# adahbingee/pais-mvs

Hardware: AMD Instinct MI355X
Metric: refined+expanded patches/sec (higher is better)
Workload: dtype f64

## Files before the change

include/pais_hip.h:

```cpp
#ifndef PAIS_HIP_H
#define PAIS_HIP_H

#include <stdint.h>
#include <stddef.h>

#ifdef __cplusplus
extern "C" {
#endif

#define PAIS_MAX_LEVELS 16
#define PAIS_MAX_VIS    64
#define PAIS_MAX_PARTICLES 128

#define PAIS_TYPE_SEED   0
#define PAIS_TYPE_EXPAND 1

typedef struct pais_config {
    int32_t cellSize;
    int32_t patchRadius;
    int32_t patchSize;
    int32_t minCamNum;
    double  textureVariation;
    double  visibleCorrelation;
    double  minCorrelation;
// ... 104 lines not shown
#define PAIS_COST_BACKFACING  1
#define PAIS_COST_OFF_IMAGE   2
#define PAIS_COST_WINDOW      3
#define PAIS_COST_OVERFLOW    4
#define PAIS_COST_ALL_MASKED  5
#define PAIS_PIX_COUNTED      0
#define PAIS_PIX_MASKED       1
#define PAIS_PIX_OVERFLOW     2
#define PAIS_PIX_NONE         3

typedef struct pais_cost_detail {
    double  fitness;
    double  sum_weight;
    double  sum_weighted_sad;
    double  pt[2];
    int32_t outcome, nx, ny;
    int32_t live_pixels;
    int32_t overflow_pixel;
    int32_t overflow_cam;
    int32_t ref_pos, _pad;
} pais_cost_detail;

int  pais_fitness_detail(pais_ctx *ctx, int n_states, const pais_patch_state *states,
                         int n_evals, const int32_t *state_index, const double *particles,
                         pais_cost_detail *out, double *weight, double *avg_sad, int8_t *pixel_code,
                         double *colour, double *homographies, int cam_stride);
int  pais_get_detail_stats(pais_ctx *ctx, double *kernel_ms, int64_t *launches, int64_t *evals, int reset);
size_t pais_sizeof_cost_detail(void);

int  pais_refine_batch(pais_ctx *ctx, int n, const pais_candidate *cands, pais_patch_result *out);
int  pais_refine_batch_view(pais_ctx *ctx, int n, const pais_candidate *cands, const pais_patch_result **view);
int  pais_refine_batch_begin(pais_ctx *ctx, int n, const pais_candidate *cands);
int  pais_refine_batch_end(pais_ctx *ctx, const pais_patch_result **view);

typedef struct pais_pso_run_info {
    double  range_l[3], range_u[3];
    double  init[3];
    double  ray[3];
    int32_t run;
    int32_t ref_cam, lod, num_cam;
    int32_t n_particles, max_iteration;
    int32_t iterations;
    int32_t _pad;
    int32_t cam_idx[PAIS_MAX_VIS];
} pais_pso_run_info;

typedef struct pais_pso_iter {
    double  gbest_fitness, gbest[3];
    double  iw;
    double  dispersion, velocity;
    int32_t g_idx, iteration, ended, _pad;
} pais_pso_iter;

int  pais_pso_trace_shape(pais_ctx *ctx, int n, const pais_candidate *cands, int *rows_per_run, int *particles_per_row);
int  pais_pso_trace(pais_ctx *ctx, int n, const pais_candidate *cands, int max_runs, pais_patch_result *out,
                    pais_pso_run_info *runs, pais_pso_iter *iters, double *particles);
int  pais_get_trace_stats(pais_ctx *ctx, double *kernel_ms, int64_t *launches, int64_t *evals, int reset);
size_t pais_sizeof_pso_run_info(void);
size_t pais_sizeof_pso_iter(void);

int  pais_refine_batch_open(pais_ctx *ctx, int n, const pais_candidate *cands, int iterations);
int  pais_refine_batch_enqueue(pais_ctx *ctx, int iterations);
int  pais_ctx_fork_lane(pais_ctx *parent, pais_ctx **lane);
int  pais_ctx_set_round_hint(pais_ctx *ctx, int n_round);

int  pais_refine_batch_device(pais_ctx *ctx, int n, const pais_candidate *d_cands,
// ... 87 lines not shown
```

pais_mvs_amd/_lib.py:

```python
from __future__ import annotations

import ctypes as C
import os

from . import build as _build

MAX_LEVELS = 16
MAX_VIS = 64


class Config(C.Structure):
    _fields_ = [
        ("cellSize", C.c_int32), ("patchRadius", C.c_int32), ("patchSize", C.c_int32), ("minCamNum", C.c_int32),
        ("textureVariation", C.c_double), ("visibleCorrelation", C.c_double), ("minCorrelation", C.c_double),
        ("maxFitness", C.c_double), ("lodRatio", C.c_double),
        ("minLOD", C.c_int32), ("maxLOD", C.c_int32), ("maxCellPatchNum", C.c_int32), ("_pad0", C.c_int32),
        ("reduceNormalRange", C.c_double),
        ("adaptiveDistanceEnable", C.c_int32), ("adaptiveDifferenceEnable", C.c_int32),
        ("adaptiveGradientEnable", C.c_int32), ("_pad1", C.c_int32),
        ("distWeighting", C.c_double), ("diffWeighting", C.c_double), ("gradientWeighting", C.c_double),
        ("neighborRadius", C.c_double), ("neighborRadiusScalar", C.c_double), ("minRegionRatio", C.c_double),
        ("depthRangeScalar", C.c_double),
        ("particleNum", C.c_int32), ("maxIteration", C.c_int32), ("expansionStrategy", C.c_int32), ("_pad2", C.c_int32),
    ]
# ... 107 lines not shown
    L.pais_last_error.restype = C.c_char_p
    for n in ("pais_sizeof_config", "pais_sizeof_camera_desc", "pais_sizeof_candidate", "pais_sizeof_patch_result",
              "pais_sizeof_view_state", "pais_sizeof_view_result", "pais_sizeof_cost_detail",
              "pais_sizeof_pso_run_info", "pais_sizeof_pso_iter"):
        getattr(L, n).restype = C.c_size_t
    assert L.pais_sizeof_config() == C.sizeof(Config), (L.pais_sizeof_config(), C.sizeof(Config))
    assert L.pais_sizeof_camera_desc() == C.sizeof(CameraDesc)
    assert L.pais_sizeof_candidate() == C.sizeof(Candidate)
    assert L.pais_sizeof_patch_result() == C.sizeof(PatchResult), (L.pais_sizeof_patch_result(), C.sizeof(PatchResult))
    assert L.pais_sizeof_view_state() == C.sizeof(ViewState), (L.pais_sizeof_view_state(), C.sizeof(ViewState))
    assert L.pais_sizeof_view_result() == C.sizeof(ViewResult), (L.pais_sizeof_view_result(), C.sizeof(ViewResult))
    assert L.pais_sizeof_cost_detail() == C.sizeof(CostDetail), (L.pais_sizeof_cost_detail(), C.sizeof(CostDetail))
    assert L.pais_sizeof_pso_run_info() == C.sizeof(PsoRunInfo), (L.pais_sizeof_pso_run_info(), C.sizeof(PsoRunInfo))
    assert L.pais_sizeof_pso_iter() == C.sizeof(PsoIter), (L.pais_sizeof_pso_iter(), C.sizeof(PsoIter))
    L.pais_ctx_create.restype = C.c_int
    L.pais_ctx_create.argtypes = [C.POINTER(Config), C.c_int, C.POINTER(CameraDesc), C.c_int, C.c_uint64,
                                  C.POINTER(C.c_void_p)]
    L.pais_ctx_set_config.argtypes = [C.c_void_p, C.POINTER(Config)]
    L.pais_ctx_set_neighbor_radius.argtypes = [C.c_void_p, C.c_double]
    L.pais_ctx_destroy.argtypes = [C.c_void_p]
    L.pais_ctx_destroy.restype = None
    L.pais_ctx_stream.restype = C.c_void_p
    L.pais_ctx_stream.argtypes = [C.c_void_p]
    L.pais_ctx_synchronize.argtypes = [C.c_void_p]
    L.pais_fitness_batch.argtypes = [C.c_void_p, C.c_int, C.POINTER(PatchState), C.c_int, C.POINTER(C.c_int32),
                                     C.POINTER(C.c_double), C.POINTER(C.c_double)]
    L.pais_refine_batch.argtypes = [C.c_void_p, C.c_int, C.POINTER(Candidate), C.POINTER(PatchResult)]
    L.pais_refine_batch_device.argtypes = [C.c_void_p, C.c_int, C.c_void_p, C.c_void_p, C.c_int, C.c_int]
    L.pais_refine_batch_begin.argtypes = [C.c_void_p, C.c_int, C.POINTER(Candidate)]
    L.pais_refine_batch_open.argtypes = [C.c_void_p, C.c_int, C.POINTER(Candidate), C.c_int]
    L.pais_refine_batch_enqueue.argtypes = [C.c_void_p, C.c_int]
    L.pais_ctx_set_round_hint.argtypes = [C.c_void_p, C.c_int]
    L.pais_refine_batch_end.argtypes = [C.c_void_p, C.POINTER(C.POINTER(PatchResult))]
    L.pais_ctx_fork_lane.argtypes = [C.c_void_p, C.POINTER(C.c_void_p)]
    L.pais_get_kernel_stats.argtypes = [C.c_void_p, C.POINTER(KernelStats), C.c_int]
    L.pais_ctx_set_fine_timing.argtypes = [C.c_void_p, C.c_int]
    L.pais_neighbor_count.argtypes = [C.c_void_p, C.c_int, C.POINTER(C.c_double), C.c_double, C.POINTER(C.c_int32), C.POINTER(C.c_double)]
    L.pais_ncc_batch.argtypes = [C.c_void_p, C.c_int, C.POINTER(ViewState), C.POINTER(ViewResult), C.POINTER(C.c_double), C.c_int]
    L.pais_fitness_detail.argtypes = [C.c_void_p, C.c_int, C.POINTER(PatchState), C.c_int, C.POINTER(C.c_int32),
                                      C.POINTER(C.c_double), C.POINTER(CostDetail), C.POINTER(C.c_double), C.POINTER(C.c_double),
                                      C.POINTER(C.c_int8), C.POINTER(C.c_double), C.POINTER(C.c_double), C.c_int]
    L.pais_pso_trace.argtypes = [C.c_void_p, C.c_int, C.POINTER(Candidate), C.c_int, C.POINTER(PatchResult), C.c_void_p, C.c_void_p,
                                 C.POINTER(C.c_double)]
    L.pais_pso_trace_shape.argtypes = [C.c_void_p, C.c_int, C.POINTER(Candidate), C.POINTER(C.c_int), C.POINTER(C.c_int)]
    L.pais_get_trace_stats.argtypes = [C.c_void_p, C.POINTER(C.c_double), C.POINTER(C.c_int64), C.POINTER(C.c_int64), C.c_int]
    L.pais_get_detail_stats.argtypes = [C.c_void_p, C.POINTER(C.c_double), C.POINTER(C.c_int64), C.POINTER(C.c_int64), C.c_int]
    L.pais_get_ncc_stats.argtypes = [C.c_void_p, C.POINTER(C.c_double), C.POINTER(C.c_int64), C.POINTER(C.c_int64), C.c_int]
    L.pais_rand31.restype = C.c_uint32
    L.pais_rand31.argtypes = [C.c_uint64, C.c_uint64, C.c_uint32, C.c_uint32]
    L.pais_child_key.restype = C.c_uint64
    L.pais_child_key.argtypes = [C.c_uint64, C.c_int, C.c_int, C.c_int]
    _lib = L
    return L


def check(rc: int, what: str = ""):
    if rc != 0:
        raise RuntimeError("%s failed (%d): %s" % (what or "pais call", rc, load().pais_last_error().decode()))
```

pais_mvs_amd/csrc/pais_capi.hip:

```cpp
#include <hip/hip_runtime.h>
#include <limits.h>
#include <math.h>
#include <stdarg.h>
#include <stddef.h>
#include <stdio.h>
#include <stdlib.h>
#include <string.h>

#include <string>
#include <utility>
#include <vector>
#include <algorithm>

#include "../../include/pais_hip.h"
#include "pais_dev.hpp"
#include "pais_host.hpp"
#include "pais_internal.h"

static thread_local std::string g_err;
static int fail(const char *what, hipError_t e)
{
    char buf[512];
    snprintf(buf, sizeof(buf), "%s: %s", what, hipGetErrorString(e));
    g_err = buf;
// ... 132 lines not shown
    DevBuf<double> d_nbC;
    DevBuf<int32_t> d_nbN;
    bool fineTiming = false;
    std::vector<EventPair> evPso, evBegin, evAfter, evEval, evEval2;
    std::vector<EventPair> evFree;
    double psoMs = 0, beginMs = 0, afterMs = 0, evalMs = 0, eval2Ms = 0;
    hipEvent_t refEv = nullptr;
    std::vector<std::pair<float, float>> eval2Intervals;
    int64_t psoLaunches = 0, evalLaunches = 0, eval2Launches = 0, tileLaunches = 0, ringLaunches = 0;
    pais_ctx *parent = nullptr;
    std::vector<pais_ctx *> lanes;
    int openBatch = -1;
    double ringPerCam = 1843.0;
    int ringMode = 1;
    int preMode = 1;
    DevBuf<double> d_pre;
    DevBuf<unsigned> d_ring;
    DevBuf<unsigned> d_ringCtl;
    PinBuf<unsigned> h_ringCtl;
    DevBuf<int> d_arrive;
    bool ringUsed = false;
    bool ringSuppressed = false;
    bool ringSuppressOnce = false;
    int ringPendingN = 0;
    double ringTimeoutMs = 10000.0;
    long ringSeedAbove = 0;
    size_t ringMaxBytes = (size_t)512 << 20;
    int64_t ringFallbacks = 0;
    std::vector<EventPair> evRing;
    double ringMs = 0;
    PassPlan plan;
    bool planDone = true;
    int roundHint = 0;
};

static void build_gauss(const pais_config &cfg, std::vector<double> &g)
{
    const int S = cfg.patchSize, r = cfg.patchRadius;
    g.assign((size_t)S * S, 0.0);
    const double sigma = cfg.distWeighting;
    const double s2 = 1.0 / (2.0 * sigma * sigma);
    const double s = 1.0 / (2.0 * M_PI * sigma * sigma);
    for (int x = 0; x < S; ++x)
        for (int y = 0; y < S; ++y) {
            double e = -(pow((double)(x - r), 2) + pow((double)(y - r), 2)) * s2;
            g[(size_t)x * S + y] = s * exp(e);
        }
    double n = 0;
    for (size_t i = 0; i < g.size(); ++i) n += g[i];
    const double inv = 1.0 / n;
    for (size_t i = 0; i < g.size(); ++i) g[i] = g[i] * inv;
}

static int apply_config(pais_ctx *ctx, const pais_config *cfg)
{
    pais_config c = *cfg;
    c.patchSize = (c.patchRadius << 1) + 1;
    if (c.patchRadius < 1 || c.patchRadius > 127) return fail_msg("patchRadius out of range");
    if (c.particleNum < 1 || c.particleNum * 2 > PAIS_MAX_PARTICLES) return fail_msg("particleNum out of range");
    if (c.maxLOD < 0 || c.maxLOD >= PAIS_MAX_LEVELS) return fail_msg("maxLOD out of range");
    std::vector<double> g;
    build_gauss(c, g);
    if (ctx->d_gauss) HIPCHK(hipStreamSynchronize(ctx->stream));
    HIPCHK(ctx->d_gauss.alloc(g.size() * sizeof(double)));
    HIPCHK(hipMemcpy(ctx->d_gauss, g.data(), g.size() * sizeof(double), hipMemcpyHostToDevice));
    ctx->sc.cfg = c;
// ... 187 lines not shown
    HIPCHK(ctx->d_stat.alloc(sizeof(unsigned long long) * 24));
    HIPCHK(hipMemset(ctx->d_stat, 0, sizeof(unsigned long long) * 24));
    ctx->stat = ctx->d_stat;
    HIPCHK(ctx->h_counters.alloc(sizeof(int) * 4));
    HIPCHK(ctx->d_ringCtl.alloc(PAIS_RING_CTL_BYTES * PAIS_RINGS));
    HIPCHK(hipMemset(ctx->d_ringCtl, 0, PAIS_RING_CTL_BYTES * PAIS_RINGS));
    HIPCHK(ctx->h_ringCtl.alloc(PAIS_RING_CTL_BYTES * PAIS_RINGS));
    memset(ctx->h_ringCtl, 0, PAIS_RING_CTL_BYTES * PAIS_RINGS);
    ctx->splitAbove = 3L * ctx->numCUs * 12;
    env_int("PAIS_EVAL_PARTS", ctx->evalParts, 1, 4);
    if (ctx->evalParts == 3) ctx->evalParts = 0;
    env_real("PAIS_PART_FILL", ctx->partFill, true);
    env_int("PAIS_SPLIT_ABOVE", ctx->splitAbove, 1);
    env_int("PAIS_PSO_MINPER", ctx->psoMinPer, 1, INT_MAX);
    env_int("PAIS_PSO_STREAMS", ctx->psoStreams, 1, 16);
    env_int("PAIS_PSO_RING", ctx->ringMode, INT_MIN, INT_MAX);
    env_int("PAIS_PRE_SETUP", ctx->preMode, INT_MIN, INT_MAX);
    env_real("PAIS_RING_PER_CAM", ctx->ringPerCam);
    env_int("PAIS_RING_SEED_ABOVE", ctx->ringSeedAbove);
    long ringMaxMB = 0;
    env_int("PAIS_RING_MAX_MB", ringMaxMB, 1);
    if (ringMaxMB) ctx->ringMaxBytes = (size_t)ringMaxMB << 20;
    env_int("PAIS_TILE", ctx->tileMode, INT_MIN, INT_MAX);
    env_flag("PAIS_TILE_DEBUG", ctx->tileDebug);
    env_flag("PAIS_TILE_VERIFY", ctx->tileVerify);
    env_int("PAIS_TILE_STRIP2", ctx->tileStrip2, 2, INT_MAX);
    env_int("PAIS_TILE_STRIP1", ctx->tileStrip1, 1, INT_MAX);
    env_flag("PAIS_TILE_FORCE_NS1", ctx->tileForceNs1);
    env_int("PAIS_TILE_SPLIT", ctx->tileSplit, INT_MIN, INT_MAX);
    if (ctx->tileSplit < 0) ctx->tileSplit = 0;
    env_int("PAIS_TILE_STRIP_SPLIT", ctx->tileStripSplit, 1, INT_MAX);
    env_int("PAIS_TILE_ABOVE", ctx->tileAbove, 1);
    env_flag("PAIS_FINE_TIMING", ctx->fineTiming);
    if (const char *e = getenv("PAIS_ARITH")) ctx->arithLiteral = (strcmp(e, "literal") == 0);
    if (const char *e = getenv("PAIS_RING_TIMEOUT_MS")) {
        const double v = atof(e);
        if (v == 0.0 && e[0] == '0') ctx->ringTimeoutMs = 0.0;
        else if (v >= 1.0 && v <= 600000.0) ctx->ringTimeoutMs = v;
        else fprintf(stderr, "pais: PAIS_RING_TIMEOUT_MS=%s ignored (0, or 1 .. 600000 ms)\n", e);
    }
    HIPCHK(hipEventCreateWithFlags(&ctx->forkEv, hipEventDisableTiming));
    for (int i = 0; i + 1 < ctx->psoStreams; ++i) {
        hipStream_t st; hipEvent_t ev;
        HIPCHK(hipStreamCreateWithFlags(&st, hipStreamNonBlocking));
        HIPCHK(hipEventCreateWithFlags(&ev, hipEventDisableTiming));
        ctx->sub.push_back(st);
        ctx->subDone.push_back(ev);
    }
    return 0;
}

extern "C" void pais_ctx_destroy(pais_ctx *ctx)
{
    if (!ctx) return;
    (void)hipSetDevice(ctx->device);
    if (ctx->parent) {
        auto &v = ctx->parent->lanes;
        for (size_t i = 0; i < v.size(); ++i)
            if (v[i] == ctx) { v.erase(v.begin() + (long)i); break; }
        ctx->parent = nullptr;
    }
    while (!ctx->lanes.empty()) {
        pais_ctx *l = ctx->lanes.back();
        ctx->lanes.pop_back();
        l->parent = nullptr;
        pais_ctx_destroy(l);
    }
    if (ctx->stream) (void)hipStreamSynchronize(ctx->stream);
    for (auto *v : {&ctx->evPso, &ctx->evBegin, &ctx->evAfter, &ctx->evEval, &ctx->evEval2, &ctx->evRing, &ctx->evFree})
        for (auto &p : *v) { (void)hipEventDestroy(p.a); (void)hipEventDestroy(p.b); }
    for (auto st : ctx->sub) (void)hipStreamDestroy(st);
    for (auto ev : ctx->subDone) (void)hipEventDestroy(ev);
    if (ctx->forkEv) (void)hipEventDestroy(ctx->forkEv);
    if (ctx->refEv) (void)hipEventDestroy(ctx->refEv);
    pais_launch::ring_profile_print();
    if (ctx->stream) (void)hipStreamDestroy(ctx->stream);
    delete ctx;
}

extern "C" int pais_ctx_set_config(pais_ctx *ctx, const pais_config *cfg)
{
    if (!ctx || !cfg) return fail_msg("pais_ctx_set_config: bad argument");
    HIPCHK(hipSetDevice(ctx->device));
    if (cfg->adaptiveGradientEnable && !ctx->d_edge && !ctx->edgesOnTheFly)
        return fail_msg("adaptiveGradientEnable needs the gradient weighting enabled at create time (edge pyramids or their on-the-fly statistics)");
    if (ctx->parent) return fail_msg("pais_ctx_set_config: a lane takes its configuration from its parent");
    for (pais_ctx *l : ctx->lanes) HIPCHK(hipStreamSynchronize(l->stream));
    int rc = apply_config(ctx, cfg);
    if (rc) return rc;
    for (pais_ctx *l : ctx->lanes) {
        l->sc.cfg = ctx->sc.cfg;
        l->sc.gauss = ctx->sc.gauss;
        for (int i = 0; i < PAIS_MAX_LEVELS; ++i) l->sc.lodScale[i] = ctx->sc.lodScale[i];
    }
    return 0;
}

extern "C" int pais_ctx_fork_lane(pais_ctx *parent, pais_ctx **out)
{
    if (!parent || !out) return fail_msg("pais_ctx_fork_lane: bad argument");
    if (parent->parent) return fail_msg("pais_ctx_fork_lane: a lane cannot be forked");
    HIPCHK(hipSetDevice(parent->device));
// ... 484 lines not shown
            if (P.useTile) ctx->tileLaunches++;
            if (P.trace) {
                const TraceOut &t = *P.trace;
                const size_t slot0 = (size_t)q.lo * t.maxRuns;
                HIPCHK(pais_launch::pso_step_trace(sc, P.d_out + q.lo, stp, q.hi - q.lo, P.Nmax, ctx->stat, t.runs + slot0, t.iters + slot0 * t.rows,
                                                   t.particles ? t.particles + slot0 * t.rows * P.Nmax * 11 : nullptr, t.maxRuns, t.rows, q.st));
                P.trace->launches++;
            } else if (!P.useIter)
                HIPCHK(pais_launch::pso_step(sc, P.d_out + q.lo, stp, q.hi - q.lo, P.Nmax, ctx->stat, q.st, ctx->d_evalBlocks + P.EB * (size_t)q.lo,
                                             P.usePre ? (double *)((unsigned char *)ctx->d_pre.p + P.PB * (size_t)q.lo) : nullptr, P.Kmax));
        }
    }
    if (tev.a) {
        if (timed_end(ctx, tev)) return -2;
        P.trace->ev->push_back(tev);
    }
    if (itEnd > P.itNext) P.itNext = itEnd;
    return 0;
}

static int pass_join(pais_ctx *ctx, PassPlan &P)
{
    for (int sI = 1; sI < P.S; ++sI) {
        bool used = false;
        for (int k = 0; k < P.nSl; ++k) used = used || (P.sl[k].st == ctx->sub[sI - 1]);
        if (!used) continue;
        HIPCHK(hipEventRecord(ctx->subDone[sI - 1], ctx->sub[sI - 1]));
        HIPCHK(hipStreamWaitEvent(ctx->stream, ctx->subDone[sI - 1], 0));
    }
    P.S = 1;
    return 0;
}

static int pass_close(pais_ctx *ctx, PassPlan &P)
{
    const DevScene &sc = ctx->sc;
    for (int k = 0; k < P.nSl; ++k) {
        const PassPlan::Slice &q = P.sl[k];
        if (P.useIter)
            HIPCHK(pais_launch::pso_iter(sc, ctx->d_psoStates, ctx->d_active, P.cnt + 2, q.lo, q.hi, P.Nmax, P.Kmax, P.d_out,
                                         ctx->stat, P.maxIt + 1, 1, q.parts, ctx->d_evalBlocks, ctx->d_win, q.st));
    }
    if (pass_join(ctx, P)) return -2;
    if (P.tp.end()) return -2;
    ctx->psoLaunches++;
    Timed ta;
    if (ta.begin(ctx, ctx->stream, &ctx->evAfter)) return -2;
    HIPCHK(pais_launch::after(sc, P.d_out, P.n, ctx->d_hp, P.afterGrid, P.cnt, ctx->stat, P.Kmax, ctx->d_ratios, P.nextCnt, ctx->stream));
    if (ta.end()) return -2;
    return 0;
}

static int batch_setup(pais_ctx *ctx, PassPlan &P, int n, const pais_candidate *d_cands, pais_patch_result *d_out, int max_num_cam, int has_seeds)
{
    HIPCHK(hipSetDevice(ctx->device));
    const DevScene &sc = ctx->sc;
    int Kmax = max_num_cam > 0 ? max_num_cam : sc.numCams;
    if (Kmax > PAIS_MAX_VIS) Kmax = PAIS_MAX_VIS;
    if (Kmax > sc.numCams) Kmax = sc.numCams;
    if (Kmax < 1) Kmax = 1;
    const int Nmax = has_seeds ? sc.cfg.particleNum * 2 : sc.cfg.particleNum;
    const int S2 = sc.cfg.patchSize * sc.cfg.patchSize;
    const int afterGrid = n < 2048 ? n : 2048;
    {
        size_t hpNeed = (size_t)afterGrid * Kmax * S2 * sizeof(double);
        const size_t full = (size_t)2048 * Kmax * S2 * sizeof(double);
        if (hpNeed > ctx->d_hp.bytes && full < ((size_t)1 << 31)) hpNeed = full;
        HIPCHK(ctx->d_hp.reserve(ctx->stream, hpNeed));
    }
    HIPCHK(ctx->d_active.reserve(ctx->stream, sizeof(int) * (size_t)n));
    HIPCHK(ctx->d_evalBlocks.reserve(ctx->stream, pais_launch::eval_block_bytes_host(Kmax) * (size_t)n));
    HIPCHK(ctx->d_win.reserve(ctx->stream, pais_launch::win_bytes_per_candidate(sc) * (size_t)n));
    const size_t SB = pais_launch::pso_state_bytes_host(Nmax);
    HIPCHK(ctx->d_psoStates.reserve(ctx->stream, SB * (size_t)n));
    HIPCHK(ctx->d_ratios.reserve(ctx->stream, sizeof(double) * PAIS_MAX_VIS * (size_t)n));
    P.n = n;
    P.hasSeeds = has_seeds != 0;
    P.Nmax = Nmax;
    P.Kmax = Kmax;
    P.afterGrid = afterGrid;
    P.maxIt = has_seeds ? sc.cfg.maxIteration * 2 : sc.cfg.maxIteration;
    P.SB = SB;
    P.EB = pais_launch::eval_block_bytes_host(Kmax);
// ... 110 lines not shown
extern "C" int pais_wire_header_device(pais_ctx *ctx, int rank, int count, int host_rc, uint32_t user_word, void *d_header)
{
    if (!ctx || !d_header) return fail_msg("pais_wire_header_device: bad argument");
    HIPCHK(hipSetDevice(ctx->device));
    HIPCHK(pais_launch::wire_header(d_header, ctx->ringPendingN > 0 ? ctx->d_ringCtl : nullptr, ctx->ringPendingN, rank, count, host_rc, user_word, ctx->stream));
    return 0;
}

extern "C" int pais_ctx_set_round_hint(pais_ctx *ctx, int n_round)
{
    if (!ctx) return fail_msg("pais_ctx_set_round_hint: bad argument");
    ctx->roundHint = n_round > 0 ? n_round : 0;
    return 0;
}

extern "C" int pais_refine_batch_view(pais_ctx *ctx, int n, const pais_candidate *cands, const pais_patch_result **view)
{
    if (!ctx || n < 0) return fail_msg("pais_refine_batch: bad argument");
    if (n == 0) return 0;
    if (!cands || !view) return fail_msg("pais_refine_batch: null pointer");
    int rc = pais_refine_batch_begin(ctx, n, cands);
    if (rc) return rc;
    return pais_refine_batch_end(ctx, view);
}

extern "C" int pais_refine_batch_begin(pais_ctx *ctx, int n, const pais_candidate *cands)
{
    int rc = pais_refine_batch_open(ctx, n, cands, 1 << 20);
    if (rc) return rc;
    rc = pais_refine_batch_enqueue(ctx, 0);
    return rc < 0 ? rc : 0;
}

extern "C" int pais_refine_batch_enqueue(pais_ctx *ctx, int iterations)
{
    if (!ctx) return fail_msg("pais_refine_batch_enqueue: bad argument");
    if (ctx->openBatch < 0) return fail_msg("pais_refine_batch_enqueue: no batch is open on this context");
    if (ctx->planDone) return 1;
    HIPCHK(hipSetDevice(ctx->device));
    PassPlan &P = ctx->plan;
    const int itEnd = iterations > 0 && iterations < P.maxIt + 1 - P.itNext ? P.itNext + iterations : P.maxIt + 1;
    int rc = pass_iterations(ctx, P, itEnd);
    if (!rc && P.itNext <= P.maxIt) return 0;
    if (!rc) rc = pass_close(ctx, P);
    if (rc) { (void)pass_join(ctx, P); ctx->openBatch = -1; ctx->ringUsed = false; return rc; }
    ctx->countersDirty = false;
    HIPCHK(hipMemcpyAsync(ctx->h_recs, ctx->d_recs, sizeof(pais_patch_result) * (size_t)ctx->openBatch, hipMemcpyDeviceToHost, ctx->stream));
    ctx->planDone = true;
    return 1;
}

extern "C" int pais_refine_batch_end(pais_ctx *ctx, const pais_patch_result **view)
{
    if (!ctx || !view) return fail_msg("pais_refine_batch_end: bad argument");
    if (ctx->openBatch < 0) return fail_msg("pais_refine_batch_end: no batch is open on this context");
    if (!ctx->planDone) {
        const int rc = pais_refine_batch_enqueue(ctx, 0);
        if (rc < 0) return rc;
    }
    ctx->openBatch = -1;
    HIPCHK(hipSetDevice(ctx->device));
    HIPCHK(hipStreamSynchronize(ctx->stream));
    if (ring_failed(ctx, ctx->plan.n)) {
        const int n = ctx->plan.n;
        const int rc = rerun_without_ring(ctx, n, ctx->d_cands, ctx->d_recs, ctx->plan.Kmax, 0, false, ctx->roundHint);
        if (rc) return rc;
        HIPCHK(hipMemcpyAsync(ctx->h_recs, ctx->d_recs, sizeof(pais_patch_result) * (size_t)n, hipMemcpyDeviceToHost, ctx->stream));
        HIPCHK(hipStreamSynchronize(ctx->stream));
    }
    *view = ctx->h_recs;
    return 0;
}

extern "C" int pais_refine_batch_open(pais_ctx *ctx, int n, const pais_candidate *cands, int iterations)
{
    if (!ctx || n <= 0 || !cands) return fail_msg("pais_refine_batch_begin: bad argument");
    if (ctx->openBatch >= 0) return fail_msg("pais_refine_batch_begin: a batch is open on this context already");
    HIPCHK(hipSetDevice(ctx->device));
    ctx->ringUsed = false;
    int Kmax = 1, hasSeeds = 0;
    int rc = check_candidates(ctx, "pais_refine_batch", n, cands, Kmax, hasSeeds);
    if (rc) return rc;
    HIPCHK(ctx->d_cands.reserve(ctx->stream, sizeof(pais_candidate) * (size_t)n));
    HIPCHK(ctx->d_recs.reserve(ctx->stream, sizeof(pais_patch_result) * (size_t)n));
    HIPCHK(ctx->h_cands.reserve(ctx->stream, sizeof(pais_candidate) * (size_t)n));
    HIPCHK(ctx->h_recs.reserve(ctx->stream, sizeof(pais_patch_result) * (size_t)n));
    memcpy(ctx->h_cands, cands, sizeof(pais_candidate) * (size_t)n);
    HIPCHK(hipMemcpyAsync(ctx->d_cands, ctx->h_cands, sizeof(pais_candidate) * (size_t)n, hipMemcpyHostToDevice, ctx->stream));
    if (hasSeeds) {
        rc = pais_refine_batch_device(ctx, n, ctx->d_cands, ctx->d_recs, Kmax, 1);
        if (rc) return rc;
        HIPCHK(hipMemcpyAsync(ctx->h_recs, ctx->d_recs, sizeof(pais_patch_result) * (size_t)n, hipMemcpyDeviceToHost, ctx->stream));
        ctx->openBatch = n;
        ctx->planDone = true;
        return 0;
    }
    PassPlan &P = ctx->plan;
    rc = batch_setup(ctx, P, n, ctx->d_cands, ctx->d_recs, Kmax, 0);
    if (!rc) rc = pass_open(ctx, P, 0, 0);
    ctx->roundHint = 0;
    if (!rc && (rc = pass_iterations(ctx, P, iterations > 0 ? iterations : 0)) != 0) (void)pass_join(ctx, P);
    if (rc) { ctx->ringUsed = false; return rc; }
    ctx->openBatch = n;
    ctx->planDone = false;
    return 0;
}

extern "C" int pais_refine_batch(pais_ctx *ctx, int n, const pais_candidate *cands, pais_patch_result *out)
{
    if (n > 0 && !out) return fail_msg("pais_refine_batch: null pointer");
    const pais_patch_result *view = nullptr;
    int rc = pais_refine_batch_view(ctx, n, cands, &view);
// ... 281 lines not shown
```

pais_mvs_amd/csrc/pais_internal.h:

```cpp
#pragma once
#include <hip/hip_runtime.h>
#include <stdint.h>

#include "../../include/pais_hip.h"

#define PAIS_STAGE_DONE  0
#define PAIS_STAGE_PSO   1
#define PAIS_STAGE_AFTER 2
#define PAIS_STAGE_AFTER2 3
#define PAIS_STAGE_AFTER2_KEEP 4
#define PAIS_STAGE_AFTER2_SAME 7

struct DevCamera {
    double KR[9], KT[3], R[9], T[3], C[3], optN[3], focal[2], pp[2];
    int maxLOD;
    int pad;
    int w[PAIS_MAX_LEVELS], h[PAIS_MAX_LEVELS];
    uint64_t imgOff[PAIS_MAX_LEVELS];
    uint64_t edgeOff[PAIS_MAX_LEVELS];
    double edgeMin[PAIS_MAX_LEVELS], edgeMax[PAIS_MAX_LEVELS];
};

typedef float2 PaisImgT;

// ... 27 lines not shown
                   double *out, int nEvals, int Kmax, unsigned char *evalBlocks, void *win, int literal, hipStream_t stream);
hipError_t pso_eval_literal(const DevScene &sc, unsigned char *states, int n, int Nmax, int Kmax, const unsigned char *evalBlocks, hipStream_t stream);
hipError_t begin(const DevScene &sc, const pais_candidate *cands, pais_patch_result *recs, int n, unsigned char *states, int Nmax,
                 int *activeList, int *activeCount, unsigned char *evalBlocks, void *win, int Kmax, hipStream_t stream);
hipError_t neighbor_count(const double *centers, int n, double radius, int32_t *counts, hipStream_t stream);
hipError_t expand_image(const uint8_t *img, PaisImgT *out, size_t n, hipStream_t stream);
hipError_t level_edge_minmax(const uint8_t *img, int w, int h, unsigned long long *minmax, hipStream_t stream);
hipError_t pack_records(const pais_patch_result *recs, int n, int Kw, void *wire, hipStream_t stream);
hipError_t wire_header(void *header, const unsigned *ringCtl, int ringN, int rank, int count, int hostRc, uint32_t userWord, hipStream_t stream);
size_t pso_state_bytes_host(int Nmax);
hipError_t pso_init(const DevScene &sc, const pais_patch_result *recs, int n, unsigned char *states, int Nmax, int *activeList,
                    int *activeCount, unsigned char *evalBlocks, void *win, int Kmax, hipStream_t stream);
hipError_t pso_eval(const DevScene &sc, unsigned char *states, int n, int Nmax, int Kmax, const unsigned char *evalBlocks, const void *win,
                    int pendingOnly, unsigned long long *verify, hipStream_t stream, const double *pre = nullptr);
size_t pre_bytes_per_candidate(int Nmax, int Kmax);
bool pre_ring_ok(int Kmax);
void ring_profile_print();
hipError_t pso_setup0(const DevScene &sc, unsigned char *states, int n, int Nmax, int Kmax, const unsigned char *evalBlocks, double *pre,
                      hipStream_t stream);
bool tile_eligible(int Kmax);
hipError_t pso_tile(const DevScene &sc, unsigned char *states, int n, int Nmax, int Kmax, const unsigned char *evalBlocks, const void *win,
                    int strip2, int strip1, int forceNs1, int split, int stripSplit, unsigned long long *dbg, hipStream_t stream);
hipError_t pso_iter(const DevScene &sc, unsigned char *states, const int *activeList, const int *activeCount, int listLo,
                    int listHi, int Nmax, int Kmax, pais_patch_result *recs, unsigned long long *stat, int L, int finishOnly,
                    int nparts, const unsigned char *evalBlocks, const void *win, hipStream_t stream);
hipError_t pso_step(const DevScene &sc, pais_patch_result *recs, unsigned char *states, int n, int Nmax,
                    unsigned long long *stat, hipStream_t stream, const unsigned char *evalBlocks = nullptr, double *pre = nullptr, int Kmax = 1);
hipError_t pso_step_trace(const DevScene &sc, pais_patch_result *recs, unsigned char *states, int n, int Nmax, unsigned long long *stat,
                          pais_pso_run_info *runs, pais_pso_iter *iters, double *particles, int maxRuns, int rows, hipStream_t stream);
size_t ring_words(int n, int Nmax, int maxIt);
hipError_t pso_ring(const DevScene &sc, pais_patch_result *recs, unsigned char *states, int n, int Nmax, int Kmax, int maxIt,
                    const unsigned char *evalBlocks, const void *win, unsigned *ring, unsigned *ctl, int *arrive, unsigned long long *stat,
                    int waves, int phase, unsigned long long timeoutTicks, hipStream_t stream, double *pre = nullptr);
hipError_t after(const DevScene &sc, pais_patch_result *recs, int n, double *hpScratch, int grid, int *counters,
                 unsigned long long *stat, int Kmax, double *ratios, int *nextCounters, hipStream_t stream);
size_t ncc_lds_bytes(int Kmax);
hipError_t ncc_batch(const DevScene &sc, const pais_view_state *states, int n, pais_view_result *out, double *tables, int stride,
                     double *hpScratch, int grid, int Kmax, int hpInLds, hipStream_t stream);
hipError_t state_blocks(const DevScene &sc, const pais_patch_state *states, int nStates, int Kmax, unsigned char *evalBlocks, void *win,
                        hipStream_t stream);
hipError_t fitness_detail(const DevScene &sc, const int32_t *idx, const double *particles, int nEvals, int Kmax, const unsigned char *evalBlocks,
                          pais_cost_detail *rec, double *weight, double *avgSad, int8_t *code, double *colour, double *H, hipStream_t stream);
}
```

pais_mvs_amd/csrc/pais_kernels.hip:

```cpp
#include <hip/hip_runtime.h>
#include <stdint.h>
#include <stdlib.h>

#include "../../include/pais_hip.h"
#include "pais_dev.hpp"
#include "pais_internal.h"

using namespace pais;

#ifndef PAIS_NS1_WAVES
#define PAIS_NS1_WAVES 2
#endif
#ifndef PAIS_NS2_WAVES
#define PAIS_NS2_WAVES 3
#endif
#define PAIS_EVAL_BOUNDS(NS) __launch_bounds__(64, (NS) == 1 ? PAIS_NS1_WAVES : PAIS_NS2_WAVES)
#ifndef PAIS_ITER_FREE_REGS_FROM
#define PAIS_ITER_FREE_REGS_FROM 2
#endif
#define PAIS_ITER_BOUNDS(P, NS) __launch_bounds__(64, (P) >= PAIS_ITER_FREE_REGS_FROM ? 1 : ((NS) == 1 ? PAIS_NS1_WAVES : PAIS_NS2_WAVES))
#ifndef PAIS_TWO_PIXELS_MAXK
#define PAIS_TWO_PIXELS_MAXK 6
#endif

// ... 2352 lines not shown
    PAIS_SHAPE_DISPATCH(pso_ring_launch, sc, recs, states, n, Nmax, Kmax, maxIt, evalBlocks, win, ring, ctl, arrive, stat, waves, phase, timeoutTicks, pre, stream);
}
hipError_t pso_step(const DevScene &sc, pais_patch_result *recs, unsigned char *states, int n, int Nmax,
                    unsigned long long *stat, hipStream_t stream, const unsigned char *evalBlocks, double *pre, int Kmax)
{
    int grid = n < 65536 ? n : 65536;
    static LdsAttr attr;
    const size_t lds = pre ? eval_block_bytes(Kmax) + step_lds_bytes(Nmax) : sizeof(double) * (size_t)Nmax * (3 * 4 + 2);
    hipError_t e = attr.ensure((const void *)k_pso_step, lds);
    if (e != hipSuccess) return e;
    hipLaunchKernelGGL(k_pso_step, dim3(grid), dim3(64), lds, stream, sc, recs, states, n, Nmax, stat, evalBlocks, eval_block_bytes(Kmax), pre, Kmax);
    return hipGetLastError();
}
hipError_t pso_step_trace(const DevScene &sc, pais_patch_result *recs, unsigned char *states, int n, int Nmax, unsigned long long *stat,
                          pais_pso_run_info *runs, pais_pso_iter *iters, double *particles, int maxRuns, int rows, hipStream_t stream)
{
    if (n <= 0) return hipSuccess;
    const int grid = n < 65536 ? n : 65536;
    static LdsAttr attr;
    const size_t lds = sizeof(double) * (size_t)Nmax * (3 * 4 + 2);
    hipError_t e = attr.ensure((const void *)k_pso_step_trace, lds);
    if (e != hipSuccess) return e;
    StepTraceSink sink;
    sink.runs = runs;
    sink.iters = iters;
    sink.particles = particles;
    sink.maxRuns = maxRuns;
    sink.rows = rows;
    sink.NP = Nmax;
    hipLaunchKernelGGL(k_pso_step_trace, dim3(grid), dim3(64), lds, stream, sc, recs, states, n, Nmax, stat, sink);
    return hipGetLastError();
}

hipError_t after(const DevScene &sc, pais_patch_result *recs, int n, double *hpScratch, int grid, int *counters,
                 unsigned long long *stat, int Kmax, double *ratios, int *nextCounters, hipStream_t stream)
{
    if (n <= 0) return hipSuccess;
    static LdsAttr attr1, attr2;
    size_t lds = after_lds_bytes(Kmax);
    const size_t hpBytes = sizeof(double) * (size_t)Kmax * sc.cfg.patchSize * sc.cfg.patchSize;
    const int hpInLds = hpBytes <= 60 * 1024 ? 1 : 0;
    if (hpInLds) lds += hpBytes;
    hipError_t e = attr1.ensure((const void *)k_after<1>, lds);
    if (e != hipSuccess) return e;
    e = attr2.ensure((const void *)k_after<2>, lds);
    if (e != hipSuccess) return e;
    const int rgrid = (int)(((long)n * Kmax + 63) / 64);
    hipLaunchKernelGGL(k_region_ratio, dim3(rgrid), dim3(64), 0, stream, sc, recs, n, PAIS_STAGE_AFTER, ratios, Kmax);
    hipLaunchKernelGGL((k_after<1>), dim3(grid), dim3(64 * AFTER_WAVES), lds, stream, sc, recs, n, hpScratch, counters, stat, Kmax, ratios, hpInLds,
                       (int *)nullptr);
    hipLaunchKernelGGL(k_region_ratio, dim3(rgrid), dim3(64), 0, stream, sc, recs, n, PAIS_STAGE_AFTER2, ratios, Kmax);
    hipLaunchKernelGGL((k_after<2>), dim3(grid), dim3(64 * AFTER_WAVES), lds, stream, sc, recs, n, hpScratch, counters, stat, Kmax, ratios, hpInLds,
                       nextCounters);
    return hipGetLastError();
}

size_t ncc_lds_bytes(int Kmax)
{
    size_t off = (sizeof(pais_view_result) + 15) & ~(size_t)15;
    off += sizeof(double) * Kmax * Kmax;
    off += sizeof(double) * 9 * Kmax;
    off += 16;
    return off;
}
hipError_t ncc_batch(const DevScene &sc, const pais_view_state *states, int n, pais_view_result *out, double *tables, int stride,
                     double *hpScratch, int grid, int Kmax, int hpInLds, hipStream_t stream)
{
    if (n <= 0) return hipSuccess;
    static LdsAttr attr;
    size_t lds = ncc_lds_bytes(Kmax);
// ... 46 lines not shown
```

pais_mvs_amd/csrc/pais_mvs.hip:

```cpp
#include <float.h>
#include <limits.h>
#include <math.h>
#include <stdio.h>
#include <stdlib.h>
#include <string.h>

#include <algorithm>
#include <condition_variable>
#include <functional>
#include <mutex>
#include <thread>
#include <chrono>
#include <deque>
#include <queue>
#include <new>
#include <string>
#include <unordered_map>
#include <unordered_set>
#include <vector>

#include <dlfcn.h>
#include <hip/hip_runtime.h>

#include "../../include/pais_mvs.h"
// ... 212 lines not shown
    struct ShardBufs {
        pais_candidate *d_shardC = nullptr, *h_shardC = nullptr;
        pais_patch_result *d_shardR = nullptr;
        size_t shardCap = 0;
        void *d_wireS = nullptr, *d_wireAll = nullptr;
        unsigned char *h_wireAll = nullptr;
        size_t wireCap = 0;
        size_t wireSCap = 0;
        hipEvent_t packed = nullptr, done = nullptr;
        std::vector<pais_candidate> hostC;
        std::vector<pais_patch_result> hostR;
        std::vector<unsigned char> hostS, hostAll;
    } sb[PAIS_MAX_STREAM_PARTS];
    struct ShardXfer {
        ShardBufs *B = nullptr;
        pais_ctx *lane = nullptr;
        const pais_candidate *c = nullptr;
        int n = 0, per = 0, lo = 0, cnt = 0, Kb = 1, Kmax = 1, hasSeeds = 0, localRc = 0;
        size_t WB = 0, slot = 0;
        double t0 = 0;
        bool sharded = false, open = false;
        bool hostRetry = false;
        bool secondAttempt = false;
    } sx[PAIS_MAX_STREAM_PARTS];
    int injectRingRetry = 0, injectGrowthFail = 0, injectRefineFail = 0;
    int *d_hs = nullptr, *d_hsAll = nullptr, *h_hs = nullptr;
    int emuMode = 0;
    std::unordered_map<uint64_t, uint32_t> emuIndex;
    std::vector<pais_patch_result> emuRecs;
    double emuLatencyUs = 25.0;
    std::vector<HostCamera> cams;
    std::vector<HostPatch *> patches;
    int alive = 0;
    bool deepPrefetch = false;
    bool trustSceneStage = true;
    std::vector<HotPatch> hot;
    std::vector<CellMap> cellMaps;
    bool blockEnable = true;
    bool blocksValid = false;
    std::vector<CellEntry> pool;
    int freeEntry = -1;
    std::priority_queue<QItem, std::vector<QItem>, BestFirst> qBest;
    std::priority_queue<QItem, std::vector<QItem>, WorstFirst> qWorst;
    std::deque<int> qList;
    uint64_t qSeq = 0;
    long liveQueued = 0;
    double neighborRadius = 0;
    std::vector<Active> active;
    std::vector<Unit> deferred, nextDeferred;
    int curRound = -1;
    int thinFront = PAIS_DEFAULT_THIN_FRONT;
    bool queueExhausted = false;
    std::vector<Candidate> cands;
    std::vector<pais_candidate> candRecs;
    std::vector<pais_patch_result> results;
    std::vector<int> seedIds;
    bool strictTail = true;
    long truncatedVisible = 0;
    pais_mvs_stats st;
    std::vector<pais_round_log> roundLog;
    double lastEnumerateMs = 0;
    EnumPool *enumPool = nullptr;
    int enumThreads = 0;
    size_t enumThreadsAbove = 4096;
    std::vector<WorkItem> work;
    std::vector<unsigned char> workState;
// ... 418 lines not shown
    void initPriorityQueue()
    {
        qBest = decltype(qBest)();
        qWorst = decltype(qWorst)();
        qList.clear();
        qSeq = 0;
        liveQueued = 0;
        for (auto *p : patches)
            if (p) queuePush(p->id);
    }
};

static thread_local std::string g_mvs_err;
static int mfail(const char *m) { g_mvs_err = m; return -1; }

extern "C" int pais_mvs_create(const pais_config *cfg, int num_cams, const pais_camera_desc *cams, int device,
                               uint64_t pso_seed, pais_mvs **out)
{
    if (!cfg || !cams || !out || num_cams <= 0) return mfail("pais_mvs_create: bad argument");
    pais_mvs *m = new pais_mvs();
    if (const char *e = getenv("PAIS_HOST_SCENE_TEST")) m->trustSceneStage = atoi(e) == 0;
    if (const char *e = getenv("PAIS_CELL_BLOCK")) m->blockEnable = atoi(e) != 0;
    if (const char *e = getenv("PAIS_THIN_FRONT")) m->thinFront = atoi(e) < 0 ? 0 : atoi(e);
    {
        const unsigned hw = std::thread::hardware_concurrency();
        (void)hw;
        m->enumThreads = 1;
        if (const char *e = getenv("PAIS_ENUM_THREADS")) m->enumThreads = std::max(1, std::min(64, atoi(e)));
        if (const char *e = getenv("PAIS_ENUM_ABOVE")) m->enumThreadsAbove = (size_t)std::max(0, atoi(e));
    }
    if (const char *e = getenv("PAIS_SHARD_ENUM")) m->shardEnum = atoi(e) != 0 ? 1 : 0;
    if (const char *e = getenv("PAIS_SHARD_ENUM_ABOVE")) m->shardEnumAbove = (size_t)std::max(0, atoi(e));
    if (const char *e = getenv("PAIS_STREAM_ROUNDS")) m->streamRounds = atoi(e);
    if (const char *e = getenv("PAIS_STREAM_ABOVE")) m->streamAbove = (size_t)std::max(0, atoi(e));
    if (const char *e = getenv("PAIS_STREAM_HOST_MS")) m->streamHostMs = atof(e);
    if (const char *e = getenv("PAIS_STREAM_HOST_SHARE")) m->streamHostShare = atof(e);
    if (const char *e = getenv("PAIS_STREAM_HEAD")) m->streamHead = std::max(1, atoi(e));
    if (const char *e = getenv("PAIS_STREAM_SHARDED")) m->streamSharded = atoi(e) != 0 ? 1 : 0;
    if (const char *e = getenv("PAIS_STREAM_CANARY")) m->streamCanaryMode = atoi(e) != 0 ? 1 : 0;
    if (const char *e = getenv("PAIS_SHARD_STRIDED")) m->shardStrided = atoi(e) != 0;
    if (const char *e = getenv("PAIS_STREAM_FIRST")) m->streamFirst = std::max(0.0, std::min(0.9, atof(e)));
    if (const char *e = getenv("PAIS_STREAM_PARTS")) m->streamParts = std::max(2, std::min(atoi(e), PAIS_MAX_STREAM_PARTS));
    if (const char *e = getenv("PAIS_STREAM_STEP")) m->streamStep = std::max(1, atoi(e));
    if (const char *e = getenv("PAIS_STREAM_SPLIT")) { const double v = atof(e); if (v > 0 && v < 1) m->streamSplit = v; }
    memset(&m->st, 0, sizeof(m->st));
    m->cfg = *cfg;
    m->cfg.patchSize = (cfg->patchRadius << 1) + 1;
    if (device >= 0) {
        int rc = pais_ctx_create(cfg, num_cams, cams, device, pso_seed, &m->ctx);
        if (rc) { g_mvs_err = pais_last_error(); delete m; return rc; }
        m->device = device;
    }
    m->cams.resize((size_t)num_cams);
    for (int c = 0; c < num_cams; ++c) {
        const pais_camera_desc &d = cams[c];
        HostCamera &h = m->cams[c];
        h.focal[0] = d.focal[0]; h.focal[1] = d.focal[1];
        h.pp[0] = d.principle_point[0]; h.pp[1] = d.principle_point[1];
        memcpy(h.R, d.rotation, sizeof(h.R));
        memcpy(h.T, d.translation, sizeof(h.T));
        memcpy(h.C, d.center, sizeof(h.C));
        memcpy(h.optN, d.optical_normal, sizeof(h.optN));
        memcpy(h.KR, d.KR, sizeof(h.KR));
        memcpy(h.KT, d.KT, sizeof(h.KT));
        h.w0 = d.level_width[0];
        h.h0 = d.level_height[0];
// ... 1422 lines not shown
            double commitMs = 0;
            const pais_patch_result *v0 = nullptr, *v1 = nullptr;
            if (n0 > 0) {
                if (pais_refine_batch_end(m->ctx, &v0)) {
                    g_mvs_err = pais_last_error();
                    if (n1 > 0) (void)pais_refine_batch_end(m->lane1, &v1);
                    return -2;
                }
                const double t1 = now_ms();
                commit_records(m, v0, 0, n0);
                commitMs += now_ms() - t1;
            }
            if (n1 > 0 && pais_refine_batch_end(m->lane1, &v1)) { g_mvs_err = pais_last_error(); return -2; }
            const double t2 = now_ms();
            if (n1 > 0) commit_records(m, v1, n0, n);
            rc = commit_finish(m, n);
            commitMs += now_ms() - t2;
            m->st.host_commit_ms += commitMs;
            if (rc) return rc;
            const double tRef = n > 0 ? std::max(0.0, (now_ms() - tFirst) - commitMs) : 0.0;
            m->st.gpu_refine_ms += tRef;
            m->st.rounds_streamed++;
            if (n > 0) m->roundLog.push_back(pais_round_log{n, 0, 0, kmax, tRef, enumMs, commitMs});
            m->prevHostMs = enumMs + commitMs;
            m->prevGpuMs = tRef + commitMs;
            if (max_rounds > 0 && ++rounds >= max_rounds) break;
            continue;
        }
        m->results.resize((size_t)(n > 0 ? n : 1));
        const double enumMs = m->lastEnumerateMs;
        double tRef = 0;
        const int64_t shardedBefore = m->st.batches_sharded;
        int kmax = 1;
        if (n > 0) {
            for (int i = 0; i < n; ++i) kmax = std::max(kmax, c[i].num_cam);
            double t0 = now_ms();
            rc = refine_any(m, n, c, m->results.data(), 0, &recs);
            tRef = now_ms() - t0;
            m->st.gpu_refine_ms += tRef;
            if (rc) return rc;
        }
        const double t1 = now_ms();
        rc = pais_mvs_round_commit(m, n > 0 ? recs : m->results.data(), n);
        if (rc) return rc;
        const double commitMs1 = now_ms() - t1;
        if (n > 0) m->roundLog.push_back(pais_round_log{n, 0, m->st.batches_sharded > shardedBefore ? 1 : 0, kmax, tRef, enumMs, commitMs1});
        m->prevHostMs = enumMs + commitMs1;
        m->prevGpuMs = tRef;
        if (max_rounds > 0 && ++rounds >= max_rounds) break;
    }
    return pais_mvs_expansion_end(m);
}

extern "C" int pais_mvs_seeds_from_matches(pais_mvs *m, int num_cams, const pais_keypoints *kp, int num_matches,
                                           const pais_pair_match *matches, double max_dist, int *num_seeds)
{
    if (!m || !kp || num_cams != (int)m->cams.size() || num_matches < 0 || (num_matches && !matches))
        return mfail("pais_mvs_seeds_from_matches: bad argument");
    const int C = num_cams;
    for (int c = 0; c < C; ++c)
        if (kp[c].n < 0 || (kp[c].n && !kp[c].xy)) return mfail("pais_mvs_seeds_from_matches: bad keypoints");
    std::vector<double> Fs((size_t)C * C * 9, 0.0);
    {
        std::vector<pais_camera_desc> d((size_t)C);
        for (int c = 0; c < C; ++c) {
            memset(&d[c], 0, sizeof(pais_camera_desc));
// ... 183 lines not shown
```

Measured before the change: 191,200.

## Chunk the post-PSO tail so host commit overlaps remaining after-kernels and copies

Splits the final 'after' kernel and device-to-host result copy into up to four chunks, each followed by an event. A new chunked begin/end API lets the host commit each chunk's records as soon as it lands, while later chunks are still being processed on the GPU. The aim is to hide host commit time and transfer latency behind GPU work at the batch tail. In exchange it adds more kernel launches and event syncs per round, smaller after-kernel grids, and a ring-failure fallback path that reruns the whole batch.

```diff
diff --git a/include/pais_hip.h b/include/pais_hip.h
--- a/include/pais_hip.h
+++ b/include/pais_hip.h
@@ -160,6 +160,8 @@
 int  pais_refine_batch_view(pais_ctx *ctx, int n, const pais_candidate *cands, const pais_patch_result **view);
 int  pais_refine_batch_begin(pais_ctx *ctx, int n, const pais_candidate *cands);
 int  pais_refine_batch_end(pais_ctx *ctx, const pais_patch_result **view);
+int  pais_refine_batch_begin_chunked(pais_ctx *ctx, int n, const pais_candidate *cands);
+int  pais_refine_batch_end_chunk(pais_ctx *ctx, const pais_patch_result **view, int *q0, int *q1);
 
 typedef struct pais_pso_run_info {
     double  range_l[3], range_u[3];
diff --git a/pais_mvs_amd/_lib.py b/pais_mvs_amd/_lib.py
--- a/pais_mvs_amd/_lib.py
+++ b/pais_mvs_amd/_lib.py
@@ -163,6 +163,8 @@
     L.pais_refine_batch_enqueue.argtypes = [C.c_void_p, C.c_int]
     L.pais_ctx_set_round_hint.argtypes = [C.c_void_p, C.c_int]
     L.pais_refine_batch_end.argtypes = [C.c_void_p, C.POINTER(C.POINTER(PatchResult))]
+    L.pais_refine_batch_begin_chunked.argtypes = [C.c_void_p, C.c_int, C.POINTER(Candidate)]
+    L.pais_refine_batch_end_chunk.argtypes = [C.c_void_p, C.POINTER(C.POINTER(PatchResult)), C.POINTER(C.c_int), C.POINTER(C.c_int)]
     L.pais_ctx_fork_lane.argtypes = [C.c_void_p, C.POINTER(C.c_void_p)]
     L.pais_get_kernel_stats.argtypes = [C.c_void_p, C.POINTER(KernelStats), C.c_int]
     L.pais_ctx_set_fine_timing.argtypes = [C.c_void_p, C.c_int]
diff --git a/pais_mvs_amd/csrc/pais_capi.hip b/pais_mvs_amd/csrc/pais_capi.hip
--- a/pais_mvs_amd/csrc/pais_capi.hip
+++ b/pais_mvs_amd/csrc/pais_capi.hip
@@ -188,6 +188,10 @@
     PassPlan plan;
     bool planDone = true;
     int roundHint = 0;
+    int tailChunks = 0;
+    bool tailWanted = false;
+    int tailC = 1, tailNext = 0;
+    std::vector<EventPair> tailEv;
 };
 
 static void build_gauss(const pais_config &cfg, std::vector<double> &g)
@@ -441,6 +445,7 @@
     env_int("PAIS_TILE_STRIP_SPLIT", ctx->tileStripSplit, 1, INT_MAX);
     env_int("PAIS_TILE_ABOVE", ctx->tileAbove, 1);
     env_flag("PAIS_FINE_TIMING", ctx->fineTiming);
+    env_int("PAIS_TAIL_CHUNKS", ctx->tailChunks, 0, INT_MAX);
     if (const char *e = getenv("PAIS_ARITH")) ctx->arithLiteral = (strcmp(e, "literal") == 0);
     if (const char *e = getenv("PAIS_RING_TIMEOUT_MS")) {
         const double v = atof(e);
@@ -476,7 +481,7 @@
         pais_ctx_destroy(l);
     }
     if (ctx->stream) (void)hipStreamSynchronize(ctx->stream);
-    for (auto *v : {&ctx->evPso, &ctx->evBegin, &ctx->evAfter, &ctx->evEval, &ctx->evEval2, &ctx->evRing, &ctx->evFree})
+    for (auto *v : {&ctx->evPso, &ctx->evBegin, &ctx->evAfter, &ctx->evEval, &ctx->evEval2, &ctx->evRing, &ctx->evFree, &ctx->tailEv})
         for (auto &p : *v) { (void)hipEventDestroy(p.a); (void)hipEventDestroy(p.b); }
     for (auto st : ctx->sub) (void)hipStreamDestroy(st);
     for (auto ev : ctx->subDone) (void)hipEventDestroy(ev);
@@ -1027,7 +1032,7 @@
     return 0;
 }
 
-static int pass_close(pais_ctx *ctx, PassPlan &P)
+static int pass_close_pso(pais_ctx *ctx, PassPlan &P)
 {
     const DevScene &sc = ctx->sc;
     for (int k = 0; k < P.nSl; ++k) {
@@ -1039,11 +1044,23 @@
     if (pass_join(ctx, P)) return -2;
     if (P.tp.end()) return -2;
     ctx->psoLaunches++;
+    return 0;
+}
+
+static int pass_after(pais_ctx *ctx, PassPlan &P, int q0, int q1, bool last)
+{
     Timed ta;
     if (ta.begin(ctx, ctx->stream, &ctx->evAfter)) return -2;
-    HIPCHK(pais_launch::after(sc, P.d_out, P.n, ctx->d_hp, P.afterGrid, P.cnt, ctx->stat, P.Kmax, ctx->d_ratios, P.nextCnt, ctx->stream));
+    HIPCHK(pais_launch::after(ctx->sc, P.d_out, q0, q1 - q0, ctx->d_hp, P.afterGrid, P.cnt, ctx->stat, P.Kmax, ctx->d_ratios, last ? P.nextCnt : nullptr,
+                              ctx->stream));
     if (ta.end()) return -2;
     return 0;
+}
+
+static int pass_close(pais_ctx *ctx, PassPlan &P)
+{
+    const int rc = pass_close_pso(ctx, P);
+    return rc ? rc : pass_after(ctx, P, 0, P.n, true);
 }
 
 static int batch_setup(pais_ctx *ctx, PassPlan &P, int n, const pais_candidate *d_cands, pais_patch_result *d_out, int max_num_cam, int has_seeds)
@@ -1220,6 +1237,21 @@
     return rc < 0 ? rc : 0;
 }
 
+static constexpr int PAIS_TAIL_MIN_CHUNK = 768, PAIS_TAIL_MAX_CHUNKS = 4;
+static int tail_chunks(const pais_ctx *ctx, int n)
+{
+    if (!ctx->tailWanted || n <= 1) return 1;
+    const int C = ctx->tailChunks > 0 ? ctx->tailChunks : std::min(PAIS_TAIL_MAX_CHUNKS, n / PAIS_TAIL_MIN_CHUNK);
+    return C < 1 ? 1 : (C > n ? n : C);
+}
+static int tail_bound(int n, int C, int i) { return (int)((long)n * i / C); }
+static hipEvent_t tail_event(pais_ctx *ctx, int i) { return (i & 1) ? ctx->tailEv[(size_t)i / 2].b : ctx->tailEv[(size_t)i / 2].a; }
+static void tail_release(pais_ctx *ctx)
+{
+    for (auto &p : ctx->tailEv) ctx->evFree.push_back(p);
+    ctx->tailEv.clear();
+}
+
 extern "C" int pais_refine_batch_enqueue(pais_ctx *ctx, int iterations)
 {
     if (!ctx) return fail_msg("pais_refine_batch_enqueue: bad argument");
@@ -1230,12 +1262,68 @@
     const int itEnd = iterations > 0 && iterations < P.maxIt + 1 - P.itNext ? P.itNext + iterations : P.maxIt + 1;
     int rc = pass_iterations(ctx, P, itEnd);
     if (!rc && P.itNext <= P.maxIt) return 0;
-    if (!rc) rc = pass_close(ctx, P);
-    if (rc) { (void)pass_join(ctx, P); ctx->openBatch = -1; ctx->ringUsed = false; return rc; }
+    if (!rc) rc = pass_close_pso(ctx, P);
+    const int n = ctx->openBatch, C = tail_chunks(ctx, n);
+    while (!rc && (int)ctx->tailEv.size() * 2 < C - 1) {
+        EventPair p;
+        if ((rc = get_event_pair(ctx, p)) == 0) ctx->tailEv.push_back(p);
+    }
+    for (int i = 0; i < C && !rc; ++i) {
+        const int q0 = tail_bound(n, C, i), q1 = tail_bound(n, C, i + 1);
+        if ((rc = pass_after(ctx, P, q0, q1, i == C - 1)) != 0) break;
+        hipError_t e = hipMemcpyAsync(ctx->h_recs + q0, ctx->d_recs + q0, sizeof(pais_patch_result) * (size_t)(q1 - q0), hipMemcpyDeviceToHost, ctx->stream);
+        if (e == hipSuccess && i < C - 1) e = hipEventRecord(tail_event(ctx, i), ctx->stream);
+        if (e != hipSuccess) rc = fail("pais_refine_batch_enqueue: tail", e);
+    }
+    if (rc) { (void)pass_join(ctx, P); ctx->openBatch = -1; ctx->ringUsed = false; tail_release(ctx); return rc; }
     ctx->countersDirty = false;
-    HIPCHK(hipMemcpyAsync(ctx->h_recs, ctx->d_recs, sizeof(pais_patch_result) * (size_t)ctx->openBatch, hipMemcpyDeviceToHost, ctx->stream));
+    ctx->tailC = C;
     ctx->planDone = true;
     return 1;
+}
+
+extern "C" int pais_refine_batch_end_chunk(pais_ctx *ctx, const pais_patch_result **view, int *q0, int *q1)
+{
+    if (!ctx || !view || !q0 || !q1) return fail_msg("pais_refine_batch_end_chunk: bad argument");
+    if (ctx->openBatch < 0) return fail_msg("pais_refine_batch_end_chunk: no batch is open on this context");
+    if (!ctx->planDone) {
+        const int rc = pais_refine_batch_enqueue(ctx, 0);
+        if (rc < 0) return rc;
+    }
+    const int n = ctx->plan.n, C = ctx->tailC, i = ctx->tailNext;
+    bool last = i + 1 >= C;
+    hipError_t e = hipSetDevice(ctx->device);
+    if (e == hipSuccess) e = last ? hipStreamSynchronize(ctx->stream) : hipEventSynchronize(tail_event(ctx, i));
+    if (e != hipSuccess) { ctx->openBatch = -1; tail_release(ctx); return fail("pais_refine_batch_end_chunk: wait", e); }
+    *q0 = tail_bound(n, C, i);
+    *q1 = tail_bound(n, C, i + 1);
+    if (i == 0 && ring_failed(ctx, n)) {
+        int rc = 0;
+        if ((e = hipStreamSynchronize(ctx->stream)) != hipSuccess) rc = fail("pais_refine_batch_end_chunk: wait", e);
+        if (!rc) rc = rerun_without_ring(ctx, n, ctx->d_cands, ctx->d_recs, ctx->plan.Kmax, 0, false, ctx->roundHint);
+        if (!rc && (e = hipMemcpyAsync(ctx->h_recs, ctx->d_recs, sizeof(pais_patch_result) * (size_t)n, hipMemcpyDeviceToHost, ctx->stream)) != hipSuccess)
+            rc = fail("pais_refine_batch_end_chunk: copy", e);
+        if (!rc && (e = hipStreamSynchronize(ctx->stream)) != hipSuccess) rc = fail("pais_refine_batch_end_chunk: wait", e);
+        if (rc) { ctx->openBatch = -1; tail_release(ctx); return rc; }
+        *q0 = 0;
+        *q1 = n;
+        last = true;
+    }
+    *view = ctx->h_recs;
+    ctx->tailNext = i + 1;
+    if (!last) return 1;
+    ctx->openBatch = -1;
+    tail_release(ctx);
+    return 0;
+}
+
+extern "C" int pais_refine_batch_begin_chunked(pais_ctx *ctx, int n, const pais_candidate *cands)
+{
+    if (!ctx) return fail_msg("pais_refine_batch_begin: bad argument");
+    ctx->tailWanted = true;
+    const int rc = pais_refine_batch_begin(ctx, n, cands);
+    ctx->tailWanted = false;
+    return rc;
 }
 
 extern "C" int pais_refine_batch_end(pais_ctx *ctx, const pais_patch_result **view)
@@ -1247,6 +1335,7 @@
         if (rc < 0) return rc;
     }
     ctx->openBatch = -1;
+    tail_release(ctx);
     HIPCHK(hipSetDevice(ctx->device));
     HIPCHK(hipStreamSynchronize(ctx->stream));
     if (ring_failed(ctx, ctx->plan.n)) {
@@ -1266,6 +1355,8 @@
     if (ctx->openBatch >= 0) return fail_msg("pais_refine_batch_begin: a batch is open on this context already");
     HIPCHK(hipSetDevice(ctx->device));
     ctx->ringUsed = false;
+    ctx->tailC = 1;
+    ctx->tailNext = 0;
     int Kmax = 1, hasSeeds = 0;
     int rc = check_candidates(ctx, "pais_refine_batch", n, cands, Kmax, hasSeeds);
     if (rc) return rc;
diff --git a/pais_mvs_amd/csrc/pais_internal.h b/pais_mvs_amd/csrc/pais_internal.h
--- a/pais_mvs_amd/csrc/pais_internal.h
+++ b/pais_mvs_amd/csrc/pais_internal.h
@@ -83,7 +83,7 @@
 hipError_t pso_ring(const DevScene &sc, pais_patch_result *recs, unsigned char *states, int n, int Nmax, int Kmax, int maxIt,
                     const unsigned char *evalBlocks, const void *win, unsigned *ring, unsigned *ctl, int *arrive, unsigned long long *stat,
                     int waves, int phase, unsigned long long timeoutTicks, hipStream_t stream, double *pre = nullptr);
-hipError_t after(const DevScene &sc, pais_patch_result *recs, int n, double *hpScratch, int grid, int *counters,
+hipError_t after(const DevScene &sc, pais_patch_result *recs, int first, int n, double *hpScratch, int grid, int *counters,
                  unsigned long long *stat, int Kmax, double *ratios, int *nextCounters, hipStream_t stream);
 size_t ncc_lds_bytes(int Kmax);
 hipError_t ncc_batch(const DevScene &sc, const pais_view_state *states, int n, pais_view_result *out, double *tables, int stride,
diff --git a/pais_mvs_amd/csrc/pais_kernels.hip b/pais_mvs_amd/csrc/pais_kernels.hip
--- a/pais_mvs_amd/csrc/pais_kernels.hip
+++ b/pais_mvs_amd/csrc/pais_kernels.hip
@@ -2408,10 +2408,13 @@
     return hipGetLastError();
 }
 
-hipError_t after(const DevScene &sc, pais_patch_result *recs, int n, double *hpScratch, int grid, int *counters,
+hipError_t after(const DevScene &sc, pais_patch_result *recs, int first, int n, double *hpScratch, int grid, int *counters,
                  unsigned long long *stat, int Kmax, double *ratios, int *nextCounters, hipStream_t stream)
 {
     if (n <= 0) return hipSuccess;
+    recs += first;
+    ratios += (size_t)first * PAIS_MAX_VIS;
+    if (grid > n) grid = n;
     static LdsAttr attr1, attr2;
     size_t lds = after_lds_bytes(Kmax);
     const size_t hpBytes = sizeof(double) * (size_t)Kmax * sc.cfg.patchSize * sc.cfg.patchSize;
diff --git a/pais_mvs_amd/csrc/pais_mvs.hip b/pais_mvs_amd/csrc/pais_mvs.hip
--- a/pais_mvs_amd/csrc/pais_mvs.hip
+++ b/pais_mvs_amd/csrc/pais_mvs.hip
@@ -268,6 +268,7 @@
     std::vector<HostCamera> cams;
     std::vector<HostPatch *> patches;
     int alive = 0;
+    int tailChunks = 1;
     bool deepPrefetch = false;
     bool trustSceneStage = true;
     std::vector<HotPatch> hot;
@@ -752,6 +753,7 @@
     if (const char *e = getenv("PAIS_SHARD_ENUM")) m->shardEnum = atoi(e) != 0 ? 1 : 0;
     if (const char *e = getenv("PAIS_SHARD_ENUM_ABOVE")) m->shardEnumAbove = (size_t)std::max(0, atoi(e));
     if (const char *e = getenv("PAIS_STREAM_ROUNDS")) m->streamRounds = atoi(e);
+    if (const char *e = getenv("PAIS_TAIL_CHUNKS")) m->tailChunks = atoi(e) < 0 ? 1 : atoi(e);
     if (const char *e = getenv("PAIS_STREAM_ABOVE")) m->streamAbove = (size_t)std::max(0, atoi(e));
     if (const char *e = getenv("PAIS_STREAM_HOST_MS")) m->streamHostMs = atof(e);
     if (const char *e = getenv("PAIS_STREAM_HOST_SHARE")) m->streamHostShare = atof(e);
@@ -2240,6 +2242,33 @@
         double tRef = 0;
         const int64_t shardedBefore = m->st.batches_sharded;
         int kmax = 1;
+        if (n > 0 && oneGpu && m->emuMode == 0 && m->tailChunks != 1) {
+            for (int i = 0; i < n; ++i) kmax = std::max(kmax, c[i].num_cam);
+            const double t0 = now_ms();
+            double commitMs = 0, tLast = t0;
+            if (pais_refine_batch_begin_chunked(m->ctx, n, c)) { g_mvs_err = pais_last_error(); return -2; }
+            for (int more = 1; more > 0;) {
+                const pais_patch_result *v = nullptr;
+                int q0 = 0, q1 = 0;
+                more = pais_refine_batch_end_chunk(m->ctx, &v, &q0, &q1);
+                if (more < 0) { g_mvs_err = pais_last_error(); return more; }
+                tLast = now_ms();
+                commit_records(m, v + q0, q0, q1);
+                commitMs += now_ms() - tLast;
+            }
+            const double t2 = now_ms();
+            rc = commit_finish(m, n);
+            commitMs += now_ms() - t2;
+            m->st.host_commit_ms += commitMs;
+            if (rc) return rc;
+            tRef = std::max(0.0, (now_ms() - t0) - commitMs);
+            m->st.gpu_refine_ms += tRef;
+            m->roundLog.push_back(pais_round_log{n, 0, 0, kmax, tRef, enumMs, commitMs});
+            m->prevHostMs = enumMs + commitMs;
+            m->prevGpuMs = tLast - t0;
+            if (max_rounds > 0 && ++rounds >= max_rounds) break;
+            continue;
+        }
         if (n > 0) {
             for (int i = 0; i < n; ++i) kmax = std::max(kmax, c[i].num_cam);
             double t0 = now_ms();
```

Result: no change. 189,900 (-0.7%).
